# magenta/mt3

Measured on AMD Instinct MI355X. Metric: audio-seconds transcribed/sec (whole node), MT3-base, 1/2/4/8 MI355X, higher is better.
Workload: dtype f32; 1 GPU; BASELINE configs[2]: MT3 (model.gin) random-init, full encoder-decoder greedy decode, batch=256 synthetic 2.048 s segments per GPU, 1024 decode steps (no early exit), ids->tokens + host note decoding included; segments_per_gpu=256, segments_total=256, decode_steps=1024, decode_chains=1, decoding=greedy, parallelism=single GPU, graph_fallbacks=0, partition_fallbacks=0

## Files before the change

include/mt3_hip.h:

```cpp
#ifndef MT3_HIP_H_
#define MT3_HIP_H_

#include <math.h>
#include <stdint.h>

#ifdef __cplusplus
extern "C" {
#endif

typedef enum mt3_status {
  MT3_OK = 0,
  MT3_ERR_INVALID = -1,
  MT3_ERR_HIP = -2,
  MT3_ERR_CAPACITY = -3,
  MT3_ERR_MISSING = -4
} mt3_status;

const char* mt3_last_error(void);
int mt3_abi_version(void);

typedef struct mt3_frontend_config {
  int32_t sample_rate;
  int32_t hop_width;
  int32_t num_mel_bins;
// ... 12 lines not shown
                        int32_t frames_per_segment, const int32_t* h_n_frames ,
                        float* d_logmel, void* stream);
int mt3_frontend_logmel_dev(mt3_frontend* fe, const float* d_audio, int32_t n_segments,
                            int32_t frames_per_segment, const int32_t* d_n_frames ,
                            float* d_logmel, void* stream);

typedef struct mt3_resampler mt3_resampler;

int64_t mt3_resample_output_length(int64_t n_in, int32_t up, int32_t down);
int mt3_resampler_create(const double* h_taps , int64_t n_taps, int32_t up, int32_t down,
                         mt3_resampler** out);
void mt3_resampler_destroy(mt3_resampler* r);
int mt3_resampler_run(mt3_resampler* r, const float* d_in, int64_t n_in, float* d_out, int64_t out_capacity,
                      void* stream);

enum { MT3_PCM_U8 = 0, MT3_PCM_S16 = 1, MT3_PCM_S24 = 2, MT3_PCM_S32 = 3, MT3_PCM_F32 = 4, MT3_PCM_F64 = 5 };
#define MT3_PCM_MAX_CHANNELS 7

int mt3_pcm_decode(const void* d_pcm, int64_t n_frames, int32_t channels, int32_t format, float* d_out,
                   int64_t out_capacity, void* stream);
int mt3_resampler_run_pcm(mt3_resampler* r, const void* d_pcm, int64_t n_frames, int32_t channels, int32_t format,
                          float* d_out, int64_t out_capacity, void* stream);

typedef enum mt3_dtype { MT3_BF16 = 0, MT3_F32 = 1, MT3_FP8_E4M3 = 2  } mt3_dtype;

typedef struct mt3_engine_config {
  int32_t vocab_size;
  int32_t emb_dim;
  int32_t num_heads;
  int32_t head_dim;
  int32_t mlp_dim;
  int32_t num_encoder_layers;
  int32_t num_decoder_layers;
  int32_t input_depth;
  int32_t input_length;
  int32_t max_decode_len;
  int32_t max_batch;
  int32_t compute_dtype;
  int32_t decode_chains;
  int32_t kv_cache_dtype;
  int32_t dense_dtype;
  int32_t options;
} mt3_engine_config;

enum {
  MT3_OPT_SINGLE_RESIDUAL_STREAM = 1,
  MT3_OPT_ENCODER_SINGLE_RESIDUAL_STREAM = 4,
  MT3_OPT_SEPARATE_PROJECTIONS = 2,
  MT3_OPT_SEPARATE_QKV_PROJECTION = 8,
  MT3_OPT_NO_ROW_GROUPS = 16,
  MT3_OPT_ENCODER_F32_MFMA = 32,
  MT3_OPT_SPIN_WAITS = 64
};

typedef struct mt3_engine mt3_engine;

int mt3_engine_create(const mt3_engine_config* cfg, mt3_engine** out);
void mt3_engine_destroy(mt3_engine* e);
int mt3_engine_load_weight(mt3_engine* e, const char* name, const float* h_data,
                           const int64_t* shape, int32_t ndim);
int mt3_engine_finalize(mt3_engine* e);
int64_t mt3_engine_device_bytes(const mt3_engine* e);

int mt3_engine_encode(mt3_engine* e, const float* d_inputs, int32_t batch,
                      float* d_encoded_f32, void* stream);

enum {
  MT3_DECODE_NO_GRAPH = 1,
  MT3_DECODE_EARLY_EXIT = 2,
  MT3_DECODE_BEAM1 = 4,
  MT3_DECODE_SINGLE_STREAM = 8,
  MT3_DECODE_ASYNC = 16
};
#define MT3_DECODE_CHAINS(n) (((n) & 0xF) << 8)
int mt3_engine_decode(mt3_engine* e, int32_t batch, int32_t num_steps, int32_t flags,
                      int32_t* d_ids, float* d_first_logits, int32_t* h_steps_run, void* stream);
int mt3_engine_decode_wait(mt3_engine* e, int32_t* h_steps_run);

int mt3_engine_decode_beams(mt3_engine* e, int32_t batch, int32_t num_beams, int32_t num_steps, int32_t flags,
                            int32_t* d_ids, int32_t* d_all_ids, float* d_scores, int32_t* h_steps_run, void* stream);

typedef struct mt3_transcribe_stats {
  int32_t slots;
  int32_t groups;
  int32_t steps_run;
  int32_t polls;
  int32_t refills;
  int32_t starved_polls;
  int32_t encoder_chunks;
  int32_t compactions;
  int32_t used_graph;
  int32_t reserved[7];
} mt3_transcribe_stats;
int mt3_engine_transcribe(mt3_engine* e, const float* d_inputs, int32_t n_segments, int32_t num_steps, int32_t flags,
                          int32_t* d_ids, mt3_transcribe_stats* h_stats, void* stream);

int mt3_engine_transcribe_beams(mt3_engine* e, const float* d_inputs, int32_t n_segments, int32_t num_beams,
                                int32_t num_steps, int32_t flags, int32_t* d_ids, int32_t* d_all_ids ,
                                float* d_scores , mt3_transcribe_stats* h_stats, void* stream);

int mt3_engine_transcribe_draws(mt3_engine* e, const float* d_inputs, int32_t n_segments, int32_t per, int32_t num_steps,
                                int32_t flags, int32_t* d_ids , mt3_transcribe_stats* h_stats,
                                void* stream);

int mt3_engine_set_token_masks(mt3_engine* e, const uint32_t* h_masks , int32_t n_masks,
                               const int32_t* h_seg_mask , int32_t n_segments);
// ... 739 lines not shown
```

mt3_amd/_lib.py:

```python
from __future__ import annotations

import ctypes as C
import os

HERE = os.path.dirname(os.path.abspath(__file__))
LIB_PATH = os.path.join(HERE, "libmt3hip.so")

MT3_OK, MT3_ERR_INVALID, MT3_ERR_HIP, MT3_ERR_CAPACITY, MT3_ERR_MISSING = 0, -1, -2, -3, -4
MT3_BF16, MT3_F32, MT3_FP8_E4M3 = 0, 1, 2
EPI_STORE, EPI_RESID, EPI_GEGLU, EPI_POS, EPI_F32, EPI_HEADS = range(6)
DECODE_NO_GRAPH, DECODE_EARLY_EXIT, DECODE_BEAM1, DECODE_SINGLE_STREAM, DECODE_ASYNC = 1, 2, 4, 8, 16
(OPT_SINGLE_RESIDUAL_STREAM, OPT_SEPARATE_PROJECTIONS, OPT_ENCODER_SINGLE_RESIDUAL_STREAM,
 OPT_SEPARATE_QKV_PROJECTION, OPT_NO_ROW_GROUPS) = 1, 2, 4, 8, 16
OPT_ENCODER_F32_MFMA = 32
OPT_SPIN_WAITS = 64
DEBUG_SKIP_SELF_ATTN, DEBUG_SKIP_CROSS_ATTN = 1, 2
(STATUS_GRAPH_FALLBACKS, STATUS_LAST_DECODE_USED_GRAPH, STATUS_RESIDUAL_SPLIT, STATUS_KV_FP8, STATUS_Q_FOLD,
 STATUS_DENSE_FP8, STATUS_QKV_FOLD, STATUS_LAST_DECODE_GROUPS, STATUS_PARTITION_FALLBACKS,
 STATUS_LAST_DECODE_COMPACTIONS, STATUS_LAST_DECODE_FORKS, STATUS_SCORE_CHUNKS, STATUS_TOKEN_MASKS,
 STATUS_PROMPTS, STATUS_TOKEN_GRAMMAR, STATUS_SAMPLING, STATUS_NOTE_GRAMMAR, STATUS_SCORE_ENCODER_PASSES) = range(18)
SAMPLING_MAX_TOP_K, SAMPLING_MAX_VOCAB = 256, 2048
(MT3_PCM_U8, MT3_PCM_S16, MT3_PCM_S24, MT3_PCM_S32, MT3_PCM_F32, MT3_PCM_F64) = range(6)
PCM_MAX_CHANNELS = 7
MAX_BEAMS = 8
EV_SHIFT, EV_PITCH, EV_VELOCITY, EV_TIE, EV_PROGRAM, EV_DRUM = range(6)
EVENT_TYPE_NAMES = ("shift", "pitch", "velocity", "tie", "program", "drum")
SPEC_ONSETS, SPEC_NOTES, SPEC_TIES = range(3)
TIE_DROP_REDUNDANT_PROGRAMS = 1
PIANOROLL_PITCHES, PIANOROLL_MIN_NOTE_SECONDS = 128, 0.05
RENDER_TILE, RENDER_MAX_SAMPLE_RATE, RENDER_MAX_SAMPLES = 1024, 384000, 1 << 40
RENDER_RELEASE_SECONDS, RENDER_DRUM_SECONDS = 0.04, 0.15
NOTE_MATCH_MAX_RULES, NOTE_MATCH_NO_OFFSET = 16, -1.0
GRANULARITY_FULL, GRANULARITY_MIDI_CLASS, GRANULARITY_FLAT = range(3)
GRANULARITIES = {"full": GRANULARITY_FULL, "midi_class": GRANULARITY_MIDI_CLASS, "flat": GRANULARITY_FLAT}
TOKENIZE_MAX_STRIDE = 1 << 20
ALIGN_MAX_SHIFTS = 64
CONSENSUS_MAX_VOTERS, CONSENSUS_TILE, CONSENSUS_SCRATCH_WORDS_PER_NOTE = 64, 256, 4
NOTE_PREP_SUSTAIN, NOTE_PREP_TRIM, NOTE_PREP_TILE = 0, 1, 256
VELOCITY_KEYS, VELOCITY_THRESHOLDS, VELOCITY_MAX_WINDOW, VELOCITY_MAX_MEL = 129, 126, 64, 4096


class Mt3Error(RuntimeError):
    def __init__(self, code, msg):
        super().__init__("libmt3hip error %d: %s" % (code, msg))
        self.code = code


class FrontendConfig(C.Structure):
    _fields_ = [("sample_rate", C.c_int32), ("hop_width", C.c_int32), ("num_mel_bins", C.c_int32),
                ("fft_size", C.c_int32), ("lo_hz", C.c_float), ("hi_hz", C.c_float), ("table_dtype", C.c_int32)]


class EngineConfig(C.Structure):
    _fields_ = [(n, C.c_int32) for n in (
        "vocab_size", "emb_dim", "num_heads", "head_dim", "mlp_dim", "num_encoder_layers",
        "num_decoder_layers", "input_depth", "input_length", "max_decode_len", "max_batch", "compute_dtype",
        "decode_chains", "kv_cache_dtype", "dense_dtype", "options")]


class TranscribeStats(C.Structure):
    _fields_ = [(n, C.c_int32) for n in ("slots", "groups", "steps_run", "polls", "refills", "starved_polls",
                                         "encoder_chunks", "compactions", "used_graph")] + [("reserved", C.c_int32 * 7)]


class EventRange(C.Structure):
    _fields_ = [("type", C.c_int32), ("min_value", C.c_int32), ("max_value", C.c_int32)]


# ... 311 lines not shown
```

mt3_amd/csrc/engine.hip:

```cpp
#include <hip/hip_runtime.h>

#include <atomic>
#include <chrono>
#include <climits>
#include <cmath>
#include <condition_variable>
#include <cstdlib>
#include <cstring>
#include <functional>
#include <map>
#include <mutex>
#include <new>
#include <string>
#include <thread>
#include <vector>

#include "common.h"
#include "feed.h"
#include "kernels.h"
#include "mx8.h"
#include "mt3_hip.h"
#include "mt3_hip_debug.h"

namespace {

constexpr int kMaxPos = 2048;
constexpr int kMaxChains = 8;
constexpr int kForksPinned = 15;

uint16_t f32_to_bf16_bits(float f) {
  uint32_t u;
  std::memcpy(&u, &f, 4);
  if ((u & 0x7fffffffu) > 0x7f800000u) return static_cast<uint16_t>((u >> 16) | 0x40);
  u += 0x7fffu + ((u >> 16) & 1u);
  return static_cast<uint16_t>(u >> 16);
}

struct HostWeight {
  std::vector<float> data;
  std::vector<int64_t> shape;
};

struct Dense {
  void* w = nullptr;
  int N = 0, K = 0;
  void* p[3] = {};
  uint8_t *q = nullptr, *sc = nullptr;
};
constexpr int kFormPlanes = 1, kFormMx8 = 2;

struct LayerDev {
  Dense wqkv;
  Dense wo;
  Dense wq_x;
  Dense wkv_x;
  Dense wo_x;
  Dense wqkv_ext;
  Dense wo_ext;
  Dense w_fold;
  Dense wi;
  Dense wo_mlp;
  void* self_k = nullptr;
  void* self_v = nullptr;
  void* cross_kv = nullptr;
  float2* self_scale = nullptr;
  float2* cross_scale = nullptr;
};

constexpr int kVarBeam = 4, kVarForced = 8, kVarRetire = 16, kVarEos = 32, kVarStream = 64, kVarMask = 128,
              kVarPrompt = 256, kVarGrammar = 512, kVarSample = 1024, kVarNotes = 2048;
constexpr int kVarBeside = 4096;
constexpr int kVarBeams = 8192, kVarBeamsShift = 14;
constexpr int kMaxGroups = 4;
constexpr int kStageChunks = mt3feed::kStageChunks, kStageChunkCap = 64, kStageMinBatch = 8;
constexpr int kStreamPollSteps = 4;
constexpr int kThrottleWindow = 16;

struct Worker {
  std::thread th;
  std::mutex mu;
  std::condition_variable cv;
  std::function<void()> job;
  bool has_job = false, quit = false;
};

struct GroupGraph {
  int variant, batch, row0, rows, slot, max_len, chains;
  hipGraph_t graph;
  hipGraphExec_t exec;
};

struct PendingDecode {
  bool active = false;
  int posted = 0;
  int groups = 1;
  int rcs[kMaxGroups] = {};
  int ran[kMaxGroups] = {};
  bool used_graph[kMaxGroups] = {};
  std::string errs[kMaxGroups];
  bool beam1 = false;
  int batch = 0;
  int32_t* d_ids = nullptr;
  hipStream_t s = nullptr;
  int beams = 0;
  int num_steps = 0;
  int32_t* d_all_ids = nullptr;
  float* d_scores = nullptr;
};

template <typename T>
struct SegTableHost {
  T* rows = nullptr;
  int* seg = nullptr;
  size_t rows_cap = 0, seg_cap = 0;
  int n = 0;
  int stride = 0;
  bool seg_on = false;
  std::vector<int> seg_host;
  std::vector<int> stat;
  std::vector<T> rows_host;
};

}

struct mt3_engine {
  mt3_engine_config cfg{};
  std::map<std::string, HostWeight> raw;
  std::vector<void*> allocs;
  int64_t device_bytes = 0;
  bool finalized = false;
  int esize = 2;
  int kv_esize = 2;
  bool kv_fp8 = false;
  void* cross_stage = nullptr;
  bool dense_fp8 = false;
  uint8_t *x_q = nullptr, *x_sc = nullptr;
  uint8_t *attn_q = nullptr, *attn_sc = nullptr;
  uint8_t *h_q = nullptr, *h_sc = nullptr;
  uint8_t *enc_q = nullptr, *enc_sc = nullptr;

// ... 45 lines not shown
  SegTableHost<int> tp;
  mt3k::TokenGrammar gr{};
  bool gr_seen = false;
  mt3k::TokenNotes nt{};
  int* note = nullptr;
  uint32_t* nrow = nullptr;
  uint32_t* held = nullptr;
  uint32_t* cs_held = nullptr;
  SegTableHost<uint64_t> sstream;
  mt3_sampling* samp = nullptr;
  bool samp_on = false;
  bool samp_seen = false, samp_table = false;
  SegTableHost<uint64_t> sseed;
  bool seed_table = false;
  int* gram = nullptr;
  int* slot_seg = nullptr;
  int* cs_seg = nullptr;
  int* refill_plan = nullptr;
  int stream_max_len = 0;
  int stage_cap = 0;
  std::vector<void*> stage_kv;
  std::vector<float2*> stage_scale;
  float* cs_y = nullptr;
  void* cs_y_ct = nullptr;
  float* cs_y_ss = nullptr;
  float* cs_qkvf = nullptr;
  int* cs_int = nullptr;
  float* cs_beam = nullptr;
  int* cs_perm = nullptr;
  int compactions = 0;
  std::atomic<int> compactions_now{0};
  std::vector<GroupGraph> group_graphs;
  std::mutex graph_mu;
  Worker* workers[kMaxGroups] = {};
  int device = 0;
  PendingDecode pending;
  float* beam_f = nullptr;
  int* beam_len = nullptr;
  int* beam_len_row = nullptr;
  float* beam_cfg = nullptr;
  float* bk_live = nullptr;
  float* bk_fin_score = nullptr;
  int* bk_fin_step = nullptr;
  int* bk_fin_beam = nullptr;
  int* bk_fork_src = nullptr;
  int* bk_forks = nullptr;
  int* bk_par = nullptr;
  int* bk_tok = nullptr;

  hipStream_t part_stream[kMaxGroups] = {};
  hipEvent_t part_begin = nullptr;
  hipEvent_t wait_ev[kMaxGroups + 1][4] = {};
  bool spin_waits = false;
  int part_failed = 0;
  int last_groups = 1;

  int cur_batch = 0;
  hipStream_t cap_stream[8] = {};
  hipEvent_t cap_event[8] = {};

  int score_cap = 0;
  int score_Lp = 0;
  int score_chunk_req = 0;
  int score_chunks = 0;
  int score_passes = 0;
  bool score_planes = false;
  float* sc_y = nullptr;
  void* sc_y_ct = nullptr;
  float* sc_y_ss = nullptr;
  void* sc_qkv = nullptr;
  void* sc_attn = nullptr;
  void* sc_q = nullptr;
  void* sc_h = nullptr;
  float* sc_logits = nullptr;
  int* sc_tgt = nullptr;
  float* sc_tok = nullptr;

  int HD() const { return cfg.num_heads * cfg.head_dim; }
};

namespace {

using mt3k::brevity_penalty;

#define MT3_TRY(expr)           \
  do {                          \
    int _rc = (expr);           \
    if (_rc != MT3_OK) return _rc; \
  } while (0)

template <typename T>
mt3k::SegTable<T> seg_view(const SegTableHost<T>& tb, size_t seg0, const int* slot_seg) {
  return mt3k::SegTable<T>{tb.rows, tb.seg_on ? tb.seg + seg0 : nullptr, slot_seg, tb.stride};
}

template <typename T>
int fits(const SegTableHost<T>& tb, const char* who, int n, int lo, int hi, const char* whose, const char* why) {
  if (!tb.n) return MT3_OK;
  if (tb.seg_on && n > static_cast<int>(tb.seg_host.size()))
    return mt3::fail(MT3_ERR_INVALID, std::string(who) + ": more rows or segments than " + whose + " n_segments");
  for (int i = 0; i < (tb.seg_on ? n : 1); ++i) {
    const int r = tb.seg_on ? tb.seg_host[i] : 0;
    if (r >= 0 && (tb.stat[r] < lo || tb.stat[r] > hi)) return mt3::fail(MT3_ERR_INVALID, std::string(who) + why);
  }
  return MT3_OK;
}
// ... 602 lines not shown

int enqueue_chain_step(mt3_engine* e, int row0, int rows, int B_total, int skip, int chains, int k, hipStream_t s,
                       int done_slot) {
  int r0, n;
  chain_rows(rows, chains, k, &r0, &n);
  for (int op = 0, ops = chain_num_ops(e); op < ops; ++op)
    MT3_TRY(enqueue_chain_op(e, row0 + r0, n, B_total, skip, op, s, done_slot));
  return MT3_OK;
}

int enqueue_step(mt3_engine* e, int row0, int rows, int B_total, int skip, int chains, hipStream_t s, int done_slot) {
  for (int k = 0; k < chains; ++k) MT3_TRY(enqueue_chain_step(e, row0, rows, B_total, skip, chains, k, s, done_slot));
  return MT3_OK;
}

int chains_for(const mt3_engine* e, int B, int requested) {
  int n = requested > 0 ? requested : (e->cfg.decode_chains > 0 ? e->cfg.decode_chains : 1);
  if (n > kMaxChains) n = kMaxChains;
  while (n > 1 && B / n < 16) --n;
  return n;
}

}

extern "C" {

static void workers_stop(mt3_engine* e);
static void drop_group_graphs(mt3_engine* e);

int mt3_engine_create(const mt3_engine_config* cfg, mt3_engine** out) {
  if (!cfg || !out) return mt3::fail(MT3_ERR_INVALID, "mt3_engine_create: null argument");
  if (cfg->head_dim != 64) return mt3::fail(MT3_ERR_INVALID, "mt3_engine_create: head_dim must be 64");
  if (cfg->compute_dtype != MT3_BF16 && cfg->compute_dtype != MT3_F32)
    return mt3::fail(MT3_ERR_INVALID, "mt3_engine_create: compute_dtype must be MT3_BF16 or MT3_F32");
  if (cfg->input_length != 256 && cfg->input_length != 512)
    return mt3::fail(MT3_ERR_INVALID, "mt3_engine_create: input_length must be 256 (mt3) or 512 (ismir2021)");
  if (cfg->emb_dim % 128 || cfg->mlp_dim % 128 || cfg->vocab_size % 128 || cfg->input_depth % 64 ||
      (cfg->num_heads * 64) % 128)
    return mt3::fail(MT3_ERR_INVALID, "mt3_engine_create: emb/mlp/vocab/heads*64 must be multiples of 128");
  if (cfg->decode_chains < 0 || cfg->decode_chains > kMaxChains)
    return mt3::fail(MT3_ERR_INVALID, "mt3_engine_create: decode_chains must be in [0, 8]");
  if (cfg->max_batch <= 0 || cfg->max_decode_len <= 0 || cfg->max_decode_len > kMaxPos ||
      cfg->num_encoder_layers <= 0 || cfg->num_decoder_layers <= 0)
    return mt3::fail(MT3_ERR_INVALID, "mt3_engine_create: bad sizes");
  if (cfg->kv_cache_dtype != 0 && cfg->kv_cache_dtype != MT3_FP8_E4M3)
    return mt3::fail(MT3_ERR_INVALID, "mt3_engine_create: kv_cache_dtype must be 0 (= compute dtype) or MT3_FP8_E4M3");
  if (cfg->kv_cache_dtype == MT3_FP8_E4M3 && cfg->compute_dtype != MT3_BF16)
    return mt3::fail(MT3_ERR_INVALID, "mt3_engine_create: the fp8 K/V caches go with compute_dtype MT3_BF16");
  if (cfg->dense_dtype != 0 && cfg->dense_dtype != MT3_FP8_E4M3)
    return mt3::fail(MT3_ERR_INVALID, "mt3_engine_create: dense_dtype must be 0 (= compute dtype) or MT3_FP8_E4M3");
  if (cfg->dense_dtype == MT3_FP8_E4M3 && (cfg->compute_dtype != MT3_BF16 || cfg->emb_dim > 1024))
    return mt3::fail(MT3_ERR_INVALID, "mt3_engine_create: the MXFP8 dense path goes with compute_dtype MT3_BF16 and emb_dim <= 1024");
  if (cfg->options & ~(MT3_OPT_SINGLE_RESIDUAL_STREAM | MT3_OPT_SEPARATE_PROJECTIONS | MT3_OPT_ENCODER_SINGLE_RESIDUAL_STREAM |
                       MT3_OPT_SEPARATE_QKV_PROJECTION | MT3_OPT_NO_ROW_GROUPS | MT3_OPT_ENCODER_F32_MFMA | MT3_OPT_SPIN_WAITS))
    return mt3::fail(MT3_ERR_INVALID, "mt3_engine_create: unknown bit in options");
  mt3_engine* e = new (std::nothrow) mt3_engine();
  if (!e) return mt3::fail(MT3_ERR_INVALID, "out of host memory");
  e->cfg = *cfg;
  if (hipGetDevice(&e->device) != hipSuccess) {
    (void)hipGetLastError();
    e->device = 0;
  }
  e->dense_fp8 = cfg->dense_dtype == MT3_FP8_E4M3;
  e->x6 = cfg->compute_dtype == MT3_F32 && !(cfg->options & MT3_OPT_ENCODER_F32_MFMA);
  e->spin_waits = (cfg->options & MT3_OPT_SPIN_WAITS) != 0;
  e->esize = cfg->compute_dtype == MT3_BF16 ? 2 : 4;
  e->kv_fp8 = cfg->kv_cache_dtype == MT3_FP8_E4M3;
  e->kv_esize = e->kv_fp8 ? 1 : e->esize;
  *out = e;
  return MT3_OK;
}

void mt3_engine_destroy(mt3_engine* e) {
  if (!e) return;
  workers_stop(e);
  drop_group_graphs(e);
  for (int k = 0; k < kMaxChains; ++k) {
    if (e->cap_stream[k]) (void)hipStreamDestroy(e->cap_stream[k]);
    if (e->cap_event[k]) (void)hipEventDestroy(e->cap_event[k]);
  }
  for (int g = 0; g < kMaxGroups; ++g)
    if (e->part_stream[g]) (void)hipStreamDestroy(e->part_stream[g]);
  if (e->part_begin) (void)hipEventDestroy(e->part_begin);
  for (auto& pair : e->wait_ev)
    for (hipEvent_t ev : pair)
      if (ev) (void)hipEventDestroy(ev);
  if (e->h_pinned) (void)hipHostFree(e->h_pinned);
  for (void* p : e->allocs) (void)hipFree(p);
  delete e;
}

int mt3_engine_load_weight(mt3_engine* e, const char* name, const float* h_data, const int64_t* shape, int32_t ndim) {
  if (!e || !name || !h_data || !shape || ndim < 1 || ndim > 2)
    return mt3::fail(MT3_ERR_INVALID, "mt3_engine_load_weight: bad arguments");
  if (e->finalized) return mt3::fail(MT3_ERR_INVALID, "mt3_engine_load_weight: engine already finalized");
  HostWeight w;
  size_t n = 1;
  for (int i = 0; i < ndim; ++i) {
    if (shape[i] <= 0) return mt3::fail(MT3_ERR_INVALID, "mt3_engine_load_weight: bad shape");
    w.shape.push_back(shape[i]);
    n *= static_cast<size_t>(shape[i]);
  }
  w.data.assign(h_data, h_data + n);
  e->raw[name] = std::move(w);
  return MT3_OK;
}

int64_t mt3_engine_device_bytes(const mt3_engine* e) { return e ? e->device_bytes : 0; }

int mt3_engine_finalize(mt3_engine* e) {
  if (!e) return mt3::fail(MT3_ERR_INVALID, "mt3_engine_finalize: null engine");
  if (e->finalized) return MT3_OK;
  const mt3_engine_config& c = e->cfg;
  const int emb = c.emb_dim, hd = e->HD(), Bm = c.max_batch, T = c.input_length, L = c.max_decode_len;
  int rc;

  {
    const HostWeight* w = find(e, "encoder/continuous_inputs_projection/kernel", c.input_depth, emb);
// ... 311 lines not shown
  }
  Worker* w = e->workers[g];
  {
    std::lock_guard<std::mutex> lk(w->mu);
    w->job = std::move(fn);
    w->has_job = true;
  }
  w->cv.notify_all();
  return true;
}

static void worker_wait(mt3_engine* e, int g) {
  Worker* w = e->workers[g];
  if (!w) return;
  std::unique_lock<std::mutex> lk(w->mu);
  w->cv.wait(lk, [&] { return !w->has_job; });
}

static void workers_stop(mt3_engine* e) {
  for (int g = 0; g < kMaxGroups; ++g) {
    Worker* w = e->workers[g];
    if (!w) continue;
    {
      std::unique_lock<std::mutex> lk(w->mu);
      w->cv.wait(lk, [&] { return !w->has_job; });
      w->quit = true;
    }
    w->cv.notify_all();
    if (w->th.joinable()) w->th.join();
    delete w;
    e->workers[g] = nullptr;
  }
}

static void drop_group_graphs(mt3_engine* e) {
  for (GroupGraph& g : e->group_graphs) {
    if (g.exec) (void)hipGraphExecDestroy(g.exec);
    if (g.graph) (void)hipGraphDestroy(g.graph);
  }
  e->group_graphs.clear();
}

struct GroupRun {
  int row0, rows, batch, variant, num_steps, slot;
  bool early, use_graph;
  hipStream_t s;
  float* d_first_logits;
  float* d_step_logits;
  int ran;
  bool used_graph;
  int chains = 1;
};

static hipGraphExec_t group_graph(mt3_engine* e, const GroupRun& r, int rows) {
  std::lock_guard<std::mutex> lk(e->graph_mu);
  const int max_len = (r.variant & kVarStream) ? e->stream_max_len : 0;
  for (const GroupGraph& g : e->group_graphs)
    if (g.variant == r.variant && g.batch == r.batch && g.row0 == r.row0 && g.rows == rows && g.slot == r.slot &&
        g.max_len == max_len && g.chains == r.chains)
      return g.exec;
  const int n = r.chains;
  hipStream_t* cs = e->cap_stream + (n > 1 ? 0 : r.slot);
  hipError_t he = hipSuccess;
  for (int k = 0; k < n && he == hipSuccess; ++k) {
    if (!cs[k]) he = hipStreamCreateWithFlags(&cs[k], hipStreamNonBlocking);
    if (n > 1 && !e->cap_event[k] && he == hipSuccess) he = hipEventCreateWithFlags(&e->cap_event[k], hipEventDisableTiming);
  }
  if (he != hipSuccess || hipStreamBeginCapture(cs[0], hipStreamCaptureModeThreadLocal) != hipSuccess) {
    (void)hipGetLastError();
    return nullptr;
  }
  int rc = MT3_OK;
  if (n > 1) he = hipEventRecord(e->cap_event[0], cs[0]);
  for (int k = 1; k < n && he == hipSuccess; ++k) he = hipStreamWaitEvent(cs[k], e->cap_event[0], 0);
  for (int k = 0; k < n && he == hipSuccess && rc == MT3_OK; ++k)
    rc = enqueue_chain_step(e, r.row0, rows, r.batch, r.variant, n, k, cs[k], r.slot);
  for (int k = 1; k < n && he == hipSuccess && rc == MT3_OK; ++k) {
    he = hipEventRecord(e->cap_event[k], cs[k]);
    if (he == hipSuccess) he = hipStreamWaitEvent(cs[0], e->cap_event[k], 0);
  }
  hipGraph_t g = nullptr;
  hipGraphExec_t x = nullptr;
  const hipError_t end = hipStreamEndCapture(cs[0], &g);
  if (rc != MT3_OK || he != hipSuccess || end != hipSuccess || hipGraphInstantiate(&x, g, nullptr, nullptr, 0) != hipSuccess) {
    if (g) (void)hipGraphDestroy(g);
    (void)hipGetLastError();
    return nullptr;
  }
  e->group_graphs.push_back(GroupGraph{r.variant, r.batch, r.row0, rows, r.slot, max_len, n, g, x});
  return x;
}

static hipEvent_t wait_event(mt3_engine* e, int slot, int which) {
  hipEvent_t& ev = e->wait_ev[slot][which];
  if (!ev && hipEventCreateWithFlags(&ev, hipEventDisableTiming) != hipSuccess) {
    (void)hipGetLastError();
    ev = nullptr;
  }
  return ev;
}

static hipError_t sleep_until(hipEvent_t ev) {
  long nap_ns = 20000;
  for (;;) {
    const hipError_t he = hipEventQuery(ev);
    if (he != hipErrorNotReady) return he;
    (void)hipGetLastError();
    std::this_thread::sleep_for(std::chrono::nanoseconds(nap_ns));
    if (nap_ns < 200000) nap_ns += nap_ns / 2;
  }
}

static hipError_t wait_stream(mt3_engine* e, int slot, hipStream_t s) {
  hipEvent_t ev = e->spin_waits ? nullptr : wait_event(e, slot, 0);
  if (!ev) return hipStreamSynchronize(s);
  hipError_t he = hipEventRecord(ev, s);
  return he == hipSuccess ? sleep_until(ev) : he;
}

struct Throttle {
  mt3_engine* e;
  int slot;
  hipStream_t s;
  int recorded = 0;
  hipError_t tick(long t) {
    if (e->spin_waits || t % kThrottleWindow != kThrottleWindow - 1) return hipSuccess;
    hipEvent_t ev = wait_event(e, slot, 1);
    if (!ev) return hipSuccess;
    hipError_t he = hipSuccess;
    if (recorded) he = sleep_until(ev);
    if (he == hipSuccess) he = hipEventRecord(ev, s);
    recorded = 1;
    return he;
  }
};

static int compact_group(mt3_engine* e, const GroupRun& r, int cur) {
  const size_t r0 = static_cast<size_t>(r.row0);
  mt3k::CompactArgs a{};
  a.st = slot_state(e, r.row0, r.slot);
  a.in = input_row(e, r.row0);
  const size_t emb = a.in.dim, n4 = a.in.rp.q_n;
  if (r.variant & kVarBeam) {
    a.beam = beam1_state(e, r.row0, 0);
    a.s_beam = e->cs_beam + 2 * r0;
  }
  a.s_y = e->cs_y + r0 * emb;
  if (a.in.y_ct) a.s_y_ct = static_cast<char*>(e->cs_y_ct) + r0 * emb * 2;
  if (a.in.y_ss) a.s_y_ss = e->cs_y_ss + r0 * (emb / 16);
  if (a.in.rp.q_out) a.s_qkvf = e->cs_qkvf + r0 * n4;
  a.s_int = e->cs_int + mt3k::kCompactInts * r0;
  if (a.st.note) a.s_held = e->cs_held + r0 * a.st.held_words;
  a.perm = e->cs_perm + r0 + r.slot;
  a.rows = cur;
  if (r.variant & kVarStream) a.s_seg = e->cs_seg + r0;
  else a.st.slot_seg = nullptr;
  return mt3k::launch_compact(a, r.s);
}

static int run_group(mt3_engine* e, GroupRun& r) {
  const mt3_engine_config& c = e->cfg;
  const bool retire = (r.variant & kVarRetire) != 0;
  const bool whole = r.row0 == 0 && r.rows == r.batch;
  int cur = r.rows;
  hipGraphExec_t exec = nullptr;
  int exec_rows = -1;
  r.ran = 0;
  r.used_graph = r.use_graph;
  const int wslot = r.s == e->part_stream[r.slot] ? r.slot : kMaxGroups;
  Throttle throttle{e, wslot, r.s};
  for (int t = 0; t < r.num_steps; ++t) {
    if (r.use_graph && exec_rows != cur) {
      exec = group_graph(e, r, cur);
      exec_rows = cur;
      if (!exec) {
        r.use_graph = r.used_graph = false;
        ++e->graph_fallbacks;
      }
    }
    if (r.use_graph) MT3_HIP_CHECK(hipGraphLaunch(exec, r.s));
    else MT3_TRY(enqueue_step(e, r.row0, cur, r.batch, r.variant, r.chains, r.s, r.slot));
    ++r.ran;
    if (whole && t == 0 && r.d_first_logits)
      MT3_HIP_CHECK(hipMemcpyAsync(r.d_first_logits, e->logits, static_cast<size_t>(r.batch) * c.vocab_size * 4,
                                   hipMemcpyDeviceToDevice, r.s));
    if (whole && r.d_step_logits)
      MT3_HIP_CHECK(hipMemcpyAsync(r.d_step_logits + static_cast<size_t>(t) * r.batch * c.vocab_size, e->logits,
                                   static_cast<size_t>(r.batch) * c.vocab_size * 4, hipMemcpyDeviceToDevice, r.s));
    if (!r.early) MT3_HIP_CHECK(throttle.tick(t));
    if (r.early && t % 32 == 31) {
      MT3_HIP_CHECK(hipMemcpyAsync(e->h_pinned + r.slot, e->n_done + r.slot, 4, hipMemcpyDeviceToHost, r.s));
      MT3_HIP_CHECK(wait_stream(e, wslot, r.s));
      const int live = r.rows - e->h_pinned[r.slot];
      if (live <= 0) break;
      if (retire && !(r.variant & kVarBeams) && r.chains == 1) {
        int want = (live + 31) & ~31;
        if (want > r.rows) want = r.rows;
        if (want < cur) {
          MT3_TRY(compact_group(e, r, cur));
          cur = want;
          ++e->compactions_now;
        }
      }
    }
  }
  return MT3_OK;
}

static int ensure_group_streams(mt3_engine* e, int groups) {
  int n_cu = 0;
  if (hipDeviceGetAttribute(&n_cu, hipDeviceAttributeMultiprocessorCount, e->device) != hipSuccess || n_cu < 2 * groups)
    return MT3_ERR_CAPACITY;
  for (int g = 0; g < groups; ++g) {
    if (e->part_stream[g]) continue;
    std::vector<uint32_t> mask((n_cu + 31) / 32, 0u);
    for (int i = 0; i < n_cu; ++i) mask[i >> 5] |= 1u << (i & 31);
    if (hipExtStreamCreateWithCUMask(&e->part_stream[g], static_cast<uint32_t>(mask.size()), mask.data()) != hipSuccess) {
      e->part_stream[g] = nullptr;
      (void)hipGetLastError();
      return MT3_ERR_CAPACITY;
    }
  }
  if (!e->part_begin && hipEventCreateWithFlags(&e->part_begin, hipEventDisableTiming) != hipSuccess)
    return MT3_ERR_CAPACITY;
  return MT3_OK;
}

using mt3feed::Feed;
using mt3feed::FeedRange;
using mt3feed::feed_fail;
using mt3feed::feed_pop;
using mt3feed::feed_release;
using mt3feed::feed_wait;

struct GroupJob {
// ... 370 lines not shown
  x->src_batch = rg.batch;
  x->src_entry0 = rg.entry0;
  x->dst_batch = dst_batch;
  x->per = per;
}

static int refill_group(mt3_engine* e, const GroupRun& r, int cur, const FeedRange* rg, const StreamJob& sj) {
  const mt3_engine_config& c = e->cfg;
  const size_t r0 = static_cast<size_t>(r.row0);
  mt3k::RefillArgs a{};
  a.st = slot_state(e, r.row0, r.slot);
  a.in = input_row(e, r.row0);
  if (r.variant & kVarBeam) a.beam = beam1_state(e, r.row0, 0);
  a.ids = e->ids;
  a.ids_stride = c.max_decode_len;
  a.out_ids = sj.d_ids;
  a.plan = e->refill_plan + r0 + r.slot;
  a.rows = cur;
  a.gram0 = grammar_initial(e);
  if (rg) {
    a.n_new = rg->n;
    a.first_seg = rg->first_seg;
    fill_staged_cross(e, *rg, r.batch, &a.x, sj.per);
  }
  return mt3k::launch_refill(a, r.s);
}

static int refill_beam_group(mt3_engine* e, const GroupRun& r, const FeedRange* rg, const StreamJob& sj) {
  const mt3_engine_config& c = e->cfg;
  mt3k::BeamRefillArgs a{};
  a.b = beam_args(e, r.row0, r.rows, sj.unit, r.slot);
  a.plan = e->refill_plan + r.row0 + r.slot;
  a.L = c.max_decode_len;
  a.num_steps = r.num_steps;
  a.out_ids = sj.d_ids;
  a.out_all = sj.d_all_ids;
  a.out_scores = sj.d_scores;
  a.gram0 = grammar_initial(e);
  if (rg) {
    a.n_new = rg->n;
    a.first_seg = rg->first_seg;
    fill_staged_cross(e, *rg, r.batch, &a.x, sj.per);
  }
  return mt3k::launch_beam_refill(a, r.s);
}

static int run_group_stream(mt3_engine* e, GroupRun& r, Feed& f, const StreamJob& sj) {
  const bool beams = (r.variant & kVarBeams) != 0;
  const int unit = sj.unit, kPoll = sj.poll;
  auto refill = [&](int cur_rows, const FeedRange* rg) {
    return beams ? refill_beam_group(e, r, rg, sj) : refill_group(e, r, cur_rows, rg, sj);
  };
  int cur = r.rows;
  hipGraphExec_t exec = nullptr;
  int exec_rows = -1, flushed_at = -1;
  std::vector<FeedRange> held, got(kStageChunks + 2);
  r.ran = 0;
  r.used_graph = r.use_graph;
  int parity = 0;
  bool pending = false;
  const long stall_limit = static_cast<long>(r.num_steps) + 4L * kPoll + 64;
  long last_progress = 0;
  int seen_fin = 0;
  if (sj.from_ring) {
    int n_fin = r.rows;
    bool dry = false;
    while (!dry && n_fin == r.rows) {
      feed_wait(f);
      if (mt3feed::feed_failed(f)) return MT3_OK;
      const int nr = feed_pop(f, n_fin / unit, got.data(), static_cast<int>(got.size()), &dry);
      for (int i = 0; i < nr; ++i) {
        MT3_TRY(refill(cur, &got[i]));
        held.push_back(got[i]);
        n_fin -= got[i].n * unit;
      }
    }
    if (n_fin == r.rows) return MT3_OK;
    seen_fin = n_fin;
  }
  for (long t = 0;; ++t) {
    if (t - last_progress > stall_limit)
      return mt3::fail(MT3_ERR_INVALID, "mt3_engine_transcribe: a row group made no progress for num_steps + 4 polls");
    if (r.use_graph && exec_rows != cur) {
      exec = group_graph(e, r, cur);
      exec_rows = cur;
      if (!exec) {
        r.use_graph = r.used_graph = false;
        ++e->graph_fallbacks;
      }
    }
    if (r.use_graph) MT3_HIP_CHECK(hipGraphLaunch(exec, r.s));
    else MT3_TRY(enqueue_step(e, r.row0, cur, r.batch, r.variant, r.chains, r.s, r.slot));
    ++r.ran;
    if (t % kPoll != kPoll - 1) continue;
    if (pending) {
      hipEvent_t pev = wait_event(e, r.slot, 2 + (parity ^ 1));
      MT3_HIP_CHECK(e->spin_waits ? hipEventSynchronize(pev) : sleep_until(pev));
      feed_release(f, held);
      held.clear();
      int n_fin = e->h_pinned[r.slot + kMaxGroups * (parity ^ 1)];
      if (n_fin != seen_fin) last_progress = t;
      bool dry = false;
      for (;;) {
        if (mt3feed::feed_failed(f)) return MT3_OK;
        const int refillable = (n_fin - (r.rows - cur)) / unit;
        const int nr = feed_pop(f, refillable, got.data(), static_cast<int>(got.size()), &dry);
        for (int i = 0; i < nr; ++i) {
          MT3_TRY(refill(cur, &got[i]));
          held.push_back(got[i]);
          n_fin -= got[i].n * unit;
          last_progress = t;
        }
        if (dry || n_fin < r.rows) break;
        feed_wait(f);
      }
      if (dry) {
        const int live = r.rows - n_fin;
        int want = (live + 31) & ~31;
        if (want > r.rows) want = r.rows;
        const bool compact = !beams && live > 0 && want < cur;
        if ((n_fin - (r.rows - cur) > 0 && n_fin != flushed_at) || compact || live <= 0) {
          MT3_TRY(refill(cur, nullptr));
          flushed_at = n_fin;
        }
        if (live <= 0) break;
        if (compact) {
          MT3_TRY(compact_group(e, r, cur));
          cur = want;
          ++e->compactions_now;
          last_progress = t;
        }
      }
      seen_fin = n_fin;
    }
    hipEvent_t ev = wait_event(e, r.slot, 2 + parity);
    if (!ev) return mt3::fail(MT3_ERR_HIP, "mt3_engine_transcribe: could not create a poll event");
    MT3_HIP_CHECK(hipMemcpyAsync(e->h_pinned + r.slot + kMaxGroups * parity, e->n_done + r.slot, 4, hipMemcpyDeviceToHost, r.s));
    MT3_HIP_CHECK(hipEventRecord(ev, r.s));
    pending = true;
    parity ^= 1;
  }
  MT3_HIP_CHECK(wait_stream(e, r.slot, r.s));
  feed_release(f, held);
  return MT3_OK;
}

// ... 717 lines not shown
```

mt3_amd/network.py:

```python
from __future__ import annotations

import ctypes as C
import dataclasses
import math
from typing import Dict, Optional, Sequence

import numpy as np

from . import _lib


@dataclasses.dataclass(frozen=True)
class T5Config:
    vocab_size: int = 1536
    dtype: str = "bfloat16"
    emb_dim: int = 512
    num_heads: int = 6
    num_encoder_layers: int = 8
    num_decoder_layers: int = 8
    head_dim: int = 64
    mlp_dim: int = 1024
    mlp_activations: Sequence[str] = ("gelu", "linear")
    dropout_rate: float = 0.1
    logits_via_embedding: bool = False
# ... 21 lines not shown
        s[f"{p}/out/kernel"] = (hd, e)

    def mlp(p):
        s[f"{p}/wi_0/kernel"] = (e, f)
        s[f"{p}/wi_1/kernel"] = (e, f)
        s[f"{p}/wo/kernel"] = (f, e)

    for i in range(cfg.num_encoder_layers):
        p = f"encoder/layers_{i}"
        s[f"{p}/pre_attention_layer_norm/scale"] = (e,)
        attn(f"{p}/attention")
        s[f"{p}/pre_mlp_layer_norm/scale"] = (e,)
        mlp(f"{p}/mlp")
    for i in range(cfg.num_decoder_layers):
        p = f"decoder/layers_{i}"
        s[f"{p}/pre_self_attention_layer_norm/scale"] = (e,)
        attn(f"{p}/self_attention")
        s[f"{p}/pre_cross_attention_layer_norm/scale"] = (e,)
        attn(f"{p}/encoder_decoder_attention")
        s[f"{p}/pre_mlp_layer_norm/scale"] = (e,)
        mlp(f"{p}/mlp")
    return s


def init_random_params(cfg: T5Config, seed: int = 0, norm_scale_jitter: float = 0.0) -> Dict[str, np.ndarray]:
    import torch
    g = torch.Generator().manual_seed(seed)
    out = {}
    for name, shape in param_shapes(cfg).items():
        if name.endswith("/scale"):
            w = torch.ones(shape)
            if norm_scale_jitter:
                w = w + norm_scale_jitter * torch.randn(shape, generator=g)
        elif name.endswith("/embedding"):
            w = torch.randn(shape, generator=g)
        else:
            fan_in = shape[0]
            std = math.sqrt(1.0 / fan_in)
            if "/attention/" in name or "_attention/" in name:
                w = torch.randn(shape, generator=g) * std
                if name.endswith("query/kernel"):
                    w = w / math.sqrt(cfg.head_dim)
            else:
                w = torch.empty(shape)
                torch.nn.init.trunc_normal_(w, mean=0.0, std=1.0, a=-2.0, b=2.0, generator=g)
                w = w * (std / 0.87962566103423978)
        out[name] = w.numpy().astype(np.float32)
    return out


class Transformer:

    def __init__(self, config: T5Config, input_length: int = 256, max_decode_length: int = 1024,
                 max_batch: int = 8, decode_chains: int = 1, options: int = 0):
        self.config = config
        self.input_length, self.max_decode_length, self.max_batch = input_length, max_decode_length, max_batch
        if config.dtype not in ("bfloat16", "float32"):
            raise ValueError("T5Config.dtype must be 'bfloat16' or 'float32'")
        if config.kv_dtype not in ("", "fp8_e4m3") or (config.kv_dtype and config.dtype != "bfloat16"):
            raise ValueError("T5Config.kv_dtype must be '' or 'fp8_e4m3' (the latter with dtype 'bfloat16')")
        if config.dense_dtype not in ("", "fp8_e4m3") or (config.dense_dtype and config.dtype != "bfloat16"):
            raise ValueError("T5Config.dense_dtype must be '' or 'fp8_e4m3' (the latter with dtype 'bfloat16')")
        self._lib = _lib.load()
        ec = _lib.EngineConfig(config.vocab_size, config.emb_dim, config.num_heads, config.head_dim, config.mlp_dim,
                               config.num_encoder_layers, config.num_decoder_layers, config.input_depth,
                               input_length, max_decode_length, max_batch,
                               _lib.MT3_BF16 if config.dtype == "bfloat16" else _lib.MT3_F32, decode_chains,
                               _lib.MT3_FP8_E4M3 if config.kv_dtype == "fp8_e4m3" else 0,
                               _lib.MT3_FP8_E4M3 if config.dense_dtype == "fp8_e4m3" else 0, options)
        self._ec = ec
        self._h = None
        self._create()

    def _create(self):
        h = C.c_void_p()
        _lib.check(self._lib.mt3_engine_create(C.byref(self._ec), C.byref(h)))
        old, self._h = self._h, h
        if old:
            self._lib.mt3_engine_destroy(old)
        self._loaded = False

    def __del__(self):
        h, self._h = getattr(self, "_h", None), None
        if h:
            self._lib.mt3_engine_destroy(h)

    def load_params(self, params: Dict[str, np.ndarray]):
        if self._loaded:
            self._create()
        want = param_shapes(self.config)
        missing = [n for n in want if n not in params]
        if missing:
            raise _lib.Mt3Error(_lib.MT3_ERR_MISSING, "weights missing from the checkpoint: %s%s"
                                % (", ".join(missing[:4]), " ..." if len(missing) > 4 else ""))
        self.ignored_params = sorted(n for n in params if n not in want)
        H, D = self.config.num_heads, self.config.head_dim
        for name, shape in want.items():
            arr = np.asarray(params[name])
            if arr.shape != shape:
                if arr.ndim == 3 and len(shape) == 2 and (arr.shape == (shape[0], H, D) or arr.shape == (H, D, shape[1])):
                    arr = arr.reshape(shape)
                else:
                    raise _lib.Mt3Error(_lib.MT3_ERR_INVALID, "weight %s has shape %s, expected %s"
                                        % (name, tuple(arr.shape), shape))
            a = np.ascontiguousarray(arr, dtype=np.float32)
            shape = (C.c_int64 * a.ndim)(*a.shape)
            _lib.check(self._lib.mt3_engine_load_weight(self._h, name.encode(), a.ctypes.data, shape, a.ndim))
        _lib.check(self._lib.mt3_engine_finalize(self._h))
        self._loaded = True

    @property
    def device_bytes(self) -> int:
        return int(self._lib.mt3_engine_device_bytes(self._h))

    def encode(self, encoder_input_tokens, return_encoded: bool = False, num_beams: int = 1):
        import torch
        x = encoder_input_tokens
        if x.dim() != 3 or x.shape[1] != self.input_length or x.shape[2] != self.config.input_depth:
            raise ValueError(f"expected [B, {self.input_length}, {self.config.input_depth}], got {tuple(x.shape)}")
        x = x.to(device="cuda", dtype=torch.float32).contiguous()
        if num_beams < 1:
            raise ValueError(f"num_beams must be >= 1, got {num_beams}")
# ... 357 lines not shown
```

Measured before the change: 491.4 audio-s/s.

## Capture multiple decode steps per HIP graph to cut launch overhead

Decode graphs can now hold a window of consecutive steps (16 by default, set through an options field), and the step loops launch one multi-step graph whenever no host-side event such as a throttle tick, poll, logits copy or early-exit check falls inside the window. This is meant to cut per-step hipGraphLaunch cost and host round trips over the 1024 greedy steps. In exchange it captures extra, larger graphs per row count, and row compaction or polling now happens only at window boundaries.

```diff
diff --git a/include/mt3_hip.h b/include/mt3_hip.h
--- a/include/mt3_hip.h
+++ b/include/mt3_hip.h
@@ -88,6 +88,7 @@
   MT3_OPT_ENCODER_F32_MFMA = 32,
   MT3_OPT_SPIN_WAITS = 64
 };
+#define MT3_OPT_GRAPH_WINDOW(n) (((n) & 0x7F) << 8)
 
 typedef struct mt3_engine mt3_engine;
 
diff --git a/mt3_amd/_lib.py b/mt3_amd/_lib.py
--- a/mt3_amd/_lib.py
+++ b/mt3_amd/_lib.py
@@ -14,6 +14,15 @@
  OPT_SEPARATE_QKV_PROJECTION, OPT_NO_ROW_GROUPS) = 1, 2, 4, 8, 16
 OPT_ENCODER_F32_MFMA = 32
 OPT_SPIN_WAITS = 64
+GRAPH_WINDOW_DEFAULT, GRAPH_WINDOW_MAX, OPT_GRAPH_WINDOW_MASK = 16, 64, 0x7F << 8
+
+
+def opt_graph_window(n: int) -> int:
+    if not 0 <= n <= GRAPH_WINDOW_MAX:
+        raise ValueError(f"graph_window must be 0 .. {GRAPH_WINDOW_MAX}, got {n}")
+    return n << 8
+
+
 DEBUG_SKIP_SELF_ATTN, DEBUG_SKIP_CROSS_ATTN = 1, 2
 (STATUS_GRAPH_FALLBACKS, STATUS_LAST_DECODE_USED_GRAPH, STATUS_RESIDUAL_SPLIT, STATUS_KV_FP8, STATUS_Q_FOLD,
  STATUS_DENSE_FP8, STATUS_QKV_FOLD, STATUS_LAST_DECODE_GROUPS, STATUS_PARTITION_FALLBACKS,
diff --git a/mt3_amd/csrc/engine.hip b/mt3_amd/csrc/engine.hip
--- a/mt3_amd/csrc/engine.hip
+++ b/mt3_amd/csrc/engine.hip
@@ -1,5 +1,6 @@
 #include <hip/hip_runtime.h>
 
+#include <algorithm>
 #include <atomic>
 #include <chrono>
 #include <climits>
@@ -75,6 +76,7 @@
 constexpr int kStageChunks = mt3feed::kStageChunks, kStageChunkCap = 64, kStageMinBatch = 8;
 constexpr int kStreamPollSteps = 4;
 constexpr int kThrottleWindow = 16;
+constexpr int kMaxGraphWindow = 64;
 
 struct Worker {
   std::thread th;
@@ -85,7 +87,7 @@
 };
 
 struct GroupGraph {
-  int variant, batch, row0, rows, slot, max_len, chains;
+  int variant, batch, row0, rows, slot, max_len, chains, steps;
   hipGraph_t graph;
   hipGraphExec_t exec;
 };
@@ -237,6 +239,7 @@
   hipEvent_t part_begin = nullptr;
   hipEvent_t wait_ev[kMaxGroups + 1][4] = {};
   bool spin_waits = false;
+  int graph_window = kThrottleWindow;
   int part_failed = 0;
   int last_groups = 1;
 
@@ -945,8 +948,12 @@
   if (cfg->dense_dtype == MT3_FP8_E4M3 && (cfg->compute_dtype != MT3_BF16 || cfg->emb_dim > 1024))
     return mt3::fail(MT3_ERR_INVALID, "mt3_engine_create: the MXFP8 dense path goes with compute_dtype MT3_BF16 and emb_dim <= 1024");
   if (cfg->options & ~(MT3_OPT_SINGLE_RESIDUAL_STREAM | MT3_OPT_SEPARATE_PROJECTIONS | MT3_OPT_ENCODER_SINGLE_RESIDUAL_STREAM |
-                       MT3_OPT_SEPARATE_QKV_PROJECTION | MT3_OPT_NO_ROW_GROUPS | MT3_OPT_ENCODER_F32_MFMA | MT3_OPT_SPIN_WAITS))
+                       MT3_OPT_SEPARATE_QKV_PROJECTION | MT3_OPT_NO_ROW_GROUPS | MT3_OPT_ENCODER_F32_MFMA | MT3_OPT_SPIN_WAITS |
+                       MT3_OPT_GRAPH_WINDOW(0x7F)))
     return mt3::fail(MT3_ERR_INVALID, "mt3_engine_create: unknown bit in options");
+  const int graph_window = (cfg->options >> 8) & 0x7F;
+  if (graph_window > kMaxGraphWindow)
+    return mt3::fail(MT3_ERR_INVALID, "mt3_engine_create: MT3_OPT_GRAPH_WINDOW must be in [0, 64]");
   mt3_engine* e = new (std::nothrow) mt3_engine();
   if (!e) return mt3::fail(MT3_ERR_INVALID, "out of host memory");
   e->cfg = *cfg;
@@ -957,6 +964,7 @@
   e->dense_fp8 = cfg->dense_dtype == MT3_FP8_E4M3;
   e->x6 = cfg->compute_dtype == MT3_F32 && !(cfg->options & MT3_OPT_ENCODER_F32_MFMA);
   e->spin_waits = (cfg->options & MT3_OPT_SPIN_WAITS) != 0;
+  if (graph_window) e->graph_window = graph_window;
   e->esize = cfg->compute_dtype == MT3_BF16 ? 2 : 4;
   e->kv_fp8 = cfg->kv_cache_dtype == MT3_FP8_E4M3;
   e->kv_esize = e->kv_fp8 ? 1 : e->esize;
@@ -1374,12 +1382,12 @@
   int chains = 1;
 };
 
-static hipGraphExec_t group_graph(mt3_engine* e, const GroupRun& r, int rows) {
+static hipGraphExec_t group_graph(mt3_engine* e, const GroupRun& r, int rows, int steps) {
   std::lock_guard<std::mutex> lk(e->graph_mu);
   const int max_len = (r.variant & kVarStream) ? e->stream_max_len : 0;
   for (const GroupGraph& g : e->group_graphs)
     if (g.variant == r.variant && g.batch == r.batch && g.row0 == r.row0 && g.rows == rows && g.slot == r.slot &&
-        g.max_len == max_len && g.chains == r.chains)
+        g.max_len == max_len && g.chains == r.chains && g.steps == steps)
       return g.exec;
   const int n = r.chains;
   hipStream_t* cs = e->cap_stream + (n > 1 ? 0 : r.slot);
@@ -1393,13 +1401,15 @@
     return nullptr;
   }
   int rc = MT3_OK;
-  if (n > 1) he = hipEventRecord(e->cap_event[0], cs[0]);
-  for (int k = 1; k < n && he == hipSuccess; ++k) he = hipStreamWaitEvent(cs[k], e->cap_event[0], 0);
-  for (int k = 0; k < n && he == hipSuccess && rc == MT3_OK; ++k)
-    rc = enqueue_chain_step(e, r.row0, rows, r.batch, r.variant, n, k, cs[k], r.slot);
-  for (int k = 1; k < n && he == hipSuccess && rc == MT3_OK; ++k) {
-    he = hipEventRecord(e->cap_event[k], cs[k]);
-    if (he == hipSuccess) he = hipStreamWaitEvent(cs[0], e->cap_event[k], 0);
+  for (int i = 0; i < steps && he == hipSuccess && rc == MT3_OK; ++i) {
+    if (n > 1) he = hipEventRecord(e->cap_event[0], cs[0]);
+    for (int k = 1; k < n && he == hipSuccess; ++k) he = hipStreamWaitEvent(cs[k], e->cap_event[0], 0);
+    for (int k = 0; k < n && he == hipSuccess && rc == MT3_OK; ++k)
+      rc = enqueue_chain_step(e, r.row0, rows, r.batch, r.variant, n, k, cs[k], r.slot);
+    for (int k = 1; k < n && he == hipSuccess && rc == MT3_OK; ++k) {
+      he = hipEventRecord(e->cap_event[k], cs[k]);
+      if (he == hipSuccess) he = hipStreamWaitEvent(cs[0], e->cap_event[k], 0);
+    }
   }
   hipGraph_t g = nullptr;
   hipGraphExec_t x = nullptr;
@@ -1409,9 +1419,48 @@
     (void)hipGetLastError();
     return nullptr;
   }
-  e->group_graphs.push_back(GroupGraph{r.variant, r.batch, r.row0, rows, r.slot, max_len, n, g, x});
+  e->group_graphs.push_back(GroupGraph{r.variant, r.batch, r.row0, rows, r.slot, max_len, n, steps, g, x});
   return x;
 }
+
+struct GroupSteps {
+  mt3_engine* e;
+  GroupRun& r;
+  int window;
+  hipGraphExec_t exec[2] = {nullptr, nullptr};
+  int exec_rows[2] = {-1, -1};
+
+  GroupSteps(mt3_engine* e_, GroupRun& r_) : e(e_), r(r_), window(r_.use_graph ? e_->graph_window : 1) {}
+
+  hipGraphExec_t graph(int which, int cur) {
+    if (exec_rows[which] != cur) {
+      exec[which] = group_graph(e, r, cur, which ? window : 1);
+      exec_rows[which] = cur;
+      if (!exec[which]) ++e->graph_fallbacks;
+    }
+    return exec[which];
+  }
+
+  int advance(int cur, long quiet, int* n) {
+    *n = 1;
+    if (window > 1 && quiet >= window) {
+      if (hipGraphExec_t x = graph(1, cur)) {
+        MT3_HIP_CHECK(hipGraphLaunch(x, r.s));
+        *n = window;
+        return MT3_OK;
+      }
+      window = 1;
+    }
+    if (r.use_graph) {
+      if (hipGraphExec_t x = graph(0, cur)) {
+        MT3_HIP_CHECK(hipGraphLaunch(x, r.s));
+        return MT3_OK;
+      }
+      r.use_graph = r.used_graph = false;
+    }
+    return enqueue_step(e, r.row0, cur, r.batch, r.variant, r.chains, r.s, r.slot);
+  }
+};
 
 static hipEvent_t wait_event(mt3_engine* e, int slot, int which) {
   hipEvent_t& ev = e->wait_ev[slot][which];
@@ -1445,8 +1494,10 @@
   int slot;
   hipStream_t s;
   int recorded = 0;
+  int period() const { return e->graph_window > kThrottleWindow ? e->graph_window : kThrottleWindow; }
+  long quiet(long t) const { return e->spin_waits ? LONG_MAX : period() - t % period(); }
   hipError_t tick(long t) {
-    if (e->spin_waits || t % kThrottleWindow != kThrottleWindow - 1) return hipSuccess;
+    if (e->spin_waits || t % period() != period() - 1) return hipSuccess;
     hipEvent_t ev = wait_event(e, slot, 1);
     if (!ev) return hipSuccess;
     hipError_t he = hipSuccess;
@@ -1485,24 +1536,19 @@
   const bool retire = (r.variant & kVarRetire) != 0;
   const bool whole = r.row0 == 0 && r.rows == r.batch;
   int cur = r.rows;
-  hipGraphExec_t exec = nullptr;
-  int exec_rows = -1;
   r.ran = 0;
   r.used_graph = r.use_graph;
+  GroupSteps steps(e, r);
   const int wslot = r.s == e->part_stream[r.slot] ? r.slot : kMaxGroups;
   Throttle throttle{e, wslot, r.s};
-  for (int t = 0; t < r.num_steps; ++t) {
-    if (r.use_graph && exec_rows != cur) {
-      exec = group_graph(e, r, cur);
-      exec_rows = cur;
-      if (!exec) {
-        r.use_graph = r.used_graph = false;
-        ++e->graph_fallbacks;
-      }
-    }
-    if (r.use_graph) MT3_HIP_CHECK(hipGraphLaunch(exec, r.s));
-    else MT3_TRY(enqueue_step(e, r.row0, cur, r.batch, r.variant, r.chains, r.s, r.slot));
-    ++r.ran;
+  const bool first_logits = whole && r.d_first_logits, step_logits = whole && r.d_step_logits;
+  for (int t = 0, n = 0; t < r.num_steps; ++t) {
+    long quiet = r.num_steps - t;
+    if (step_logits || (first_logits && t == 0)) quiet = 1;
+    quiet = std::min(quiet, r.early ? 32L - t % 32 : throttle.quiet(t));
+    MT3_TRY(steps.advance(cur, quiet, &n));
+    r.ran += n;
+    t += n - 1;
     if (whole && t == 0 && r.d_first_logits)
       MT3_HIP_CHECK(hipMemcpyAsync(r.d_first_logits, e->logits, static_cast<size_t>(r.batch) * c.vocab_size * 4,
                                    hipMemcpyDeviceToDevice, r.s));
@@ -1979,11 +2025,11 @@
     return beams ? refill_beam_group(e, r, rg, sj) : refill_group(e, r, cur_rows, rg, sj);
   };
   int cur = r.rows;
-  hipGraphExec_t exec = nullptr;
-  int exec_rows = -1, flushed_at = -1;
+  int flushed_at = -1;
   std::vector<FeedRange> held, got(kStageChunks + 2);
   r.ran = 0;
   r.used_graph = r.use_graph;
+  GroupSteps steps(e, r);
   int parity = 0;
   bool pending = false;
   const long stall_limit = static_cast<long>(r.num_steps) + 4L * kPoll + 64;
@@ -2005,20 +2051,13 @@
     if (n_fin == r.rows) return MT3_OK;
     seen_fin = n_fin;
   }
+  int n = 0;
   for (long t = 0;; ++t) {
     if (t - last_progress > stall_limit)
       return mt3::fail(MT3_ERR_INVALID, "mt3_engine_transcribe: a row group made no progress for num_steps + 4 polls");
-    if (r.use_graph && exec_rows != cur) {
-      exec = group_graph(e, r, cur);
-      exec_rows = cur;
-      if (!exec) {
-        r.use_graph = r.used_graph = false;
-        ++e->graph_fallbacks;
-      }
-    }
-    if (r.use_graph) MT3_HIP_CHECK(hipGraphLaunch(exec, r.s));
-    else MT3_TRY(enqueue_step(e, r.row0, cur, r.batch, r.variant, r.chains, r.s, r.slot));
-    ++r.ran;
+    MT3_TRY(steps.advance(cur, kPoll - t % kPoll, &n));
+    r.ran += n;
+    t += n - 1;
     if (t % kPoll != kPoll - 1) continue;
     if (pending) {
       hipEvent_t pev = wait_event(e, r.slot, 2 + (parity ^ 1));
diff --git a/mt3_amd/network.py b/mt3_amd/network.py
--- a/mt3_amd/network.py
+++ b/mt3_amd/network.py
@@ -97,7 +97,8 @@
 class Transformer:
 
     def __init__(self, config: T5Config, input_length: int = 256, max_decode_length: int = 1024,
-                 max_batch: int = 8, decode_chains: int = 1, options: int = 0):
+                 max_batch: int = 8, decode_chains: int = 1, options: int = 0,
+                 graph_window: int = _lib.GRAPH_WINDOW_DEFAULT):
         self.config = config
         self.input_length, self.max_decode_length, self.max_batch = input_length, max_decode_length, max_batch
         if config.dtype not in ("bfloat16", "float32"):
@@ -112,7 +113,8 @@
                                input_length, max_decode_length, max_batch,
                                _lib.MT3_BF16 if config.dtype == "bfloat16" else _lib.MT3_F32, decode_chains,
                                _lib.MT3_FP8_E4M3 if config.kv_dtype == "fp8_e4m3" else 0,
-                               _lib.MT3_FP8_E4M3 if config.dense_dtype == "fp8_e4m3" else 0, options)
+                               _lib.MT3_FP8_E4M3 if config.dense_dtype == "fp8_e4m3" else 0,
+                               (options & ~_lib.OPT_GRAPH_WINDOW_MASK) | _lib.opt_graph_window(graph_window))
         self._ec = ec
         self._h = None
         self._create()
```

After: 492.6 audio-s/s, median of 5. About the same (+0.3%).
